# Danderson123/Amira

Measured on AMD Instinct MI355X. Metric: gene-mers/s to corrected GeneMerGraph, higher is better.
Workload: dtype int32; 1 GPU; synthetic 1M reads x 60 genes, k=5, 20k-gene vocab: build + error-correction sweep (build, filter(3,1), correct, build, clip(5), correct, build); reads_per_gpu=1000000, genes_per_read=60, k=5, vocab=20000, gene_mers_per_gpu=56000000, final_nodes=472478, final_edges=1054844, multi_gpu=n/a

## Files before the change

amira_amd/csrc/amg_scan.hip:

```cpp
#include "amg_rows.h"

#define SC_THREADS 512
#define SC_ROWS 16
#define SC_TILE (SC_THREADS * SC_ROWS)
#define SC_VAL_MASK ((1ull << 48) - 1ull)

__device__ __forceinline__ unsigned long long sc_word(unsigned int state, unsigned int epoch, unsigned long long v) {
  return ((unsigned long long)state << 62) | ((unsigned long long)(epoch & 0x3fffu) << 48) | (v & SC_VAL_MASK);
}

#define SC_NO_LIM 0x7fffffffffffffffll
template <class T>
struct LoadArr {
  const T* in;
  using Raw = T;
  __device__ __forceinline__ long long lim() const { return SC_NO_LIM; }
  __device__ __forceinline__ Raw raw(long long i) const { return in[i]; }
  __device__ __forceinline__ unsigned long long val(long long, Raw r) const { return (unsigned long long)r; }
};
template <class T>
struct LoadArrN {
  const T* in;
  long long n;
  using Raw = T;
  __device__ __forceinline__ long long lim() const { return n; }
  __device__ __forceinline__ Raw raw(long long i) const { return in[i]; }
  __device__ __forceinline__ unsigned long long val(long long, Raw r) const { return (unsigned long long)r; }
};
struct LoadNonzero {
  const unsigned int* in;
  long long n;
  using Raw = unsigned int;
  __device__ __forceinline__ long long lim() const { return n; }
  __device__ __forceinline__ Raw raw(long long i) const { return in[i]; }
  __device__ __forceinline__ unsigned long long val(long long, Raw r) const { return r != 0u ? 1ull : 0ull; }
};
struct LoadByteSet {
  const unsigned char* in;
  long long n;
  using Raw = unsigned char;
  __device__ __forceinline__ long long lim() const { return n; }
  __device__ __forceinline__ Raw raw(long long i) const { return in[i]; }
  __device__ __forceinline__ unsigned long long val(long long, Raw r) const { return r != 0 ? 1ull : 0ull; }
};
struct LoadApplyKill {
  unsigned char* kill;
  unsigned char* alive;
  long long n;
  struct Raw {
    unsigned int kill, alive;
  };
  __device__ __forceinline__ long long lim() const { return n; }
  __device__ __forceinline__ Raw raw(long long i) const { return Raw{kill[i], alive[i]}; }
  __device__ __forceinline__ unsigned long long val(long long i, Raw r) const {
    const bool f = r.kill != 0u && r.alive != 0u;
    if (f) alive[i] = 0;
    kill[i] = f ? 1 : 0;
    return f ? 1ull : 0ull;
  }
};
struct LoadFlagWords {
  const unsigned char* flags;
  unsigned int* bits;
  long long n_words;
  struct Raw {
    uint4 a, b;
  };
  __device__ __forceinline__ long long lim() const { return n_words; }
  __device__ __forceinline__ Raw raw(long long i) const {
    const uint4* p = reinterpret_cast<const uint4*>(flags + 32 * i);
    return Raw{p[0], p[1]};
  }
  __device__ __forceinline__ unsigned long long val(long long i, const Raw& r) const {
    auto nib = [](unsigned int x) { return (x & 1u) | ((x >> 7) & 2u) | ((x >> 14) & 4u) | ((x >> 21) & 8u); };
    const uint4 a = r.a, b = r.b;
    const unsigned int w = nib(a.x) | (nib(a.y) << 4) | (nib(a.z) << 8) | (nib(a.w) << 12) | (nib(b.x) << 16) |
                           (nib(b.y) << 20) | (nib(b.z) << 24) | (nib(b.w) << 28);
    bits[i] = w;
    return (unsigned long long)__popc(w);
  }
};
struct LoadBitsPopc {
  const unsigned int* bits;
  long long n_words;
  using Raw = unsigned int;
  __device__ __forceinline__ long long lim() const { return n_words; }
  __device__ __forceinline__ Raw raw(long long i) const { return bits[i]; }
  __device__ __forceinline__ unsigned long long val(long long, Raw r) const { return (unsigned long long)__popc(r); }
};
struct LoadPairWidth {
  const unsigned long long* pkey;
  long long n_pairs;
  using Raw = unsigned long long;
  __device__ __forceinline__ long long lim() const { return n_pairs; }
  __device__ __forceinline__ Raw raw(long long i) const { return pkey[i]; }
  __device__ __forceinline__ unsigned long long val(long long, Raw key) const {
    const unsigned int lo = (unsigned int)((key >> 32) & 0x7fffffffull);
    const unsigned int hi = (unsigned int)(key & 0xffffffffull) - 1u;
    return lo == hi ? 1ull : 2ull;
  }
};

struct LoadNone {
  using Raw = unsigned char;
  __device__ __forceinline__ long long lim() const { return 0; }
  __device__ __forceinline__ Raw raw(long long) const { return 0; }
  __device__ __forceinline__ unsigned long long val(long long, Raw) const { return 0ull; }
};

template <class L>
__device__ __forceinline__ void load_rows(const L& ld, long long w0, long long n, int lane, unsigned long long* x) {
  const long long lim = n < ld.lim() ? n : ld.lim();
  if (w0 >= lim) {
#pragma unroll
    for (int r = 0; r < SC_ROWS; ++r) x[r] = 0ull;
    return;
  }
  typename L::Raw raw[SC_ROWS];
#pragma unroll
  for (int r = 0; r < SC_ROWS; ++r) {
    const long long i = w0 + r * 64 + lane;
    raw[r] = ld.raw(i < lim ? i : lim - 1);
  }
  asm volatile("" ::: "memory");
#pragma unroll
  for (int r = 0; r < SC_ROWS; ++r) {
    const long long i = w0 + r * 64 + lane;
    x[r] = i < lim ? ld.val(i, raw[r]) : 0ull;
  }
}

struct EmitOut {
  long long* out;
  struct Pre {};
  __device__ __forceinline__ Pre pre(long long) const { return Pre{}; }
  __device__ __forceinline__ void operator()(long long i, unsigned long long excl, const Pre&, unsigned long long) const {
    out[i] = (long long)excl;
  }
};
struct EmitEdges {
  const unsigned long long* pkey;
  const unsigned int* pcnt;
  const unsigned long long* pfirst;
  long long n_pairs;
  long long* total;
  int* e_src;
  int* e_tgt;
  signed char* e_sdir;
  signed char* e_tdir;
  unsigned int* e_cov;
  unsigned char* e_alive;
  struct Pre {
    unsigned long long key, first;
    unsigned int cnt;
  };
  __device__ __forceinline__ Pre pre(long long i) const {
    const long long j = i < n_pairs ? i : 0;
    return Pre{pkey[j], pfirst[j], pcnt[j]};
  }
  __device__ __forceinline__ void operator()(long long i, unsigned long long excl, const Pre& p, unsigned long long) const {
    if (i >= n_pairs) {
      total[0] = (long long)excl;
      return;
    }
    const unsigned long long key = p.key, first = p.first;
    const int lo = (int)((key >> 32) & 0x7fffffffull);
    const int hi = (int)((key & 0xffffffffull) - 1ull);
    const int X = (first & 1ull) ? lo : hi, Y = (first & 1ull) ? hi : lo;
    const signed char dX = (first & 2ull) ? 1 : -1, dY = (first & 4ull) ? 1 : -1;
    const long long e = (long long)excl;
    const unsigned int cnt = p.cnt;
    e_src[e] = X; e_tgt[e] = Y; e_sdir[e] = dX; e_tdir[e] = dY; e_alive[e] = 1;
    if (lo == hi) {
      e_cov[e] = cnt * 2u;
    } else {
      e_cov[e] = cnt;
      e_src[e + 1] = Y; e_tgt[e + 1] = X; e_sdir[e + 1] = (signed char)-dY;
      e_tdir[e + 1] = (signed char)-dX; e_cov[e + 1] = cnt; e_alive[e + 1] = 1;
    }
  }
};
struct EmitLiveKeys {
  const int* e_src;
  const signed char* e_sdir;
  long long n_edges;
  long long* total;
  unsigned int* keys;
  unsigned int* edge_of;
  struct Pre {};
  __device__ __forceinline__ Pre pre(long long) const { return Pre{}; }
  __device__ __forceinline__ void operator()(long long i, unsigned long long excl, const Pre&, unsigned long long val) const {
    if (i >= n_edges) {
      total[0] = (long long)excl;
      return;
    }
    if (val == 0ull) return;
    keys[excl] = adj_row_of(e_src[i], e_sdir[i]);
    edge_of[excl] = (unsigned int)i;
  }
};
template <class Load, class LoadB, class Emit>
__global__ __launch_bounds__(SC_THREADS) void k_exscan(Load load, Emit emit_a, long long n_a, LoadB load_b,
                                                        long long* __restrict__ out_b, long long n_b, long long tiles_a,
                                                        unsigned long long* counter, unsigned long long ticket_base,
                                                        unsigned long long* status, unsigned int epoch, ClearArgs side) {
  __shared__ unsigned long long s_wave[SC_THREADS / 64];
  __shared__ unsigned long long s_excl;
  __shared__ unsigned int s_tile;
  const int lane = threadIdx.x & 63, wave = threadIdx.x >> 6;
  if (threadIdx.x == 0) s_tile = (unsigned int)(atomicAdd(counter, 1ull) - ticket_base);
  __syncthreads();
  const long long tile = s_tile;
  const bool second = tile >= tiles_a;
  const long long seg0 = second ? tiles_a : 0;
  const long long n = second ? n_b : n_a;
  const long long w0 = (tile - seg0) * SC_TILE + (long long)wave * (64 * SC_ROWS);
  unsigned long long x[SC_ROWS], inc[SC_ROWS];
  if (second)
    load_rows(load_b, w0, n, lane, x);
  else
    load_rows(load, w0, n, lane, x);
  unsigned long long row_off = 0;
#pragma unroll
  for (int r = 0; r < SC_ROWS; ++r) {
    unsigned long long v = x[r];
#pragma unroll
    for (int d = 1; d < 64; d <<= 1) {
      const unsigned long long o = __shfl_up(v, d, 64);
      if (lane >= d) v += o;
    }
    inc[r] = v + row_off;
    row_off += __shfl(v, 63, 64);
  }
  if (lane == 0) s_wave[wave] = row_off;
  __syncthreads();
  unsigned long long wave_excl = 0, tile_sum = 0;
#pragma unroll
  for (int w = 0; w < SC_THREADS / 64; ++w) {
    const unsigned long long s = s_wave[w];
    wave_excl += w < wave ? s : 0ull;
    tile_sum += s;
  }
  typename Emit::Pre pre[SC_ROWS];
  if (!second) {
#pragma unroll
    for (int r = 0; r < SC_ROWS; ++r) {
      const long long i = w0 + r * 64 + lane;
      pre[r] = emit_a.pre(i < n ? i : n - 1);
    }
  }
  if (wave == 0) {
    unsigned long long excl = 0;
    if (tile == seg0) {
      if (lane == 0)
        __hip_atomic_store(status + tile, sc_word(2u, epoch, tile_sum), __ATOMIC_RELAXED, __HIP_MEMORY_SCOPE_AGENT);
    } else {
      if (lane == 0)
        __hip_atomic_store(status + tile, sc_word(1u, epoch, tile_sum), __ATOMIC_RELAXED, __HIP_MEMORY_SCOPE_AGENT);
      for (long long look = tile - 1;; look -= 64) {
        const long long idx = look - lane;
        unsigned int state = 2u;
        unsigned long long val = 0;
        if (idx >= seg0) {
          unsigned long long w;
          do {
            w = __hip_atomic_load(status + idx, __ATOMIC_RELAXED, __HIP_MEMORY_SCOPE_AGENT);
          } while ((unsigned int)((w >> 48) & 0x3fffu) != (epoch & 0x3fffu) || (w >> 62) == 0ull);
          state = (unsigned int)(w >> 62);
          val = w & SC_VAL_MASK;
        }
        const unsigned long long full = __ballot(state == 2u);
        const int stop = full ? __ffsll((long long)full) - 1 : 63;
        unsigned long long part = lane <= stop ? val : 0ull;
#pragma unroll
        for (int d = 32; d > 0; d >>= 1) part += __shfl_xor(part, d, 64);
        excl += part;
        if (full) break;
      }
      if (lane == 0)
        __hip_atomic_store(status + tile, sc_word(2u, epoch, excl + tile_sum), __ATOMIC_RELAXED, __HIP_MEMORY_SCOPE_AGENT);
    }
    if (lane == 0) s_excl = excl;
  }
  __syncthreads();
  const unsigned long long base = s_excl + wave_excl;
#pragma unroll
  for (int r = 0; r < SC_ROWS; ++r) {
    const long long i = w0 + r * 64 + lane;
    if (i < n) {
      if (second)
        out_b[i] = (long long)(base + inc[r] - x[r]);
      else
        emit_a(i, base + inc[r] - x[r], pre[r], x[r]);
    }
  }
  if (side.n) clear_args_part(side, blockIdx.x, gridDim.x);
}

template <class Load, class Emit, class LoadB = LoadNone>
static int exscan_emit(amg_ctx* c, Load load, Emit emit, size_t n, LoadB load_b = LoadNone{}, long long* out_b = nullptr,
                       size_t n_b = 0, const ClearList* side = nullptr) {
  if (side && side->overflow) return amg_fail(AMG_E_ARG, "exscan: more than %d ranges in one list", CLEAR_MAX);
  if (n == 0 && n_b == 0) return side ? clear_many(c, *side) : AMG_OK;
  const unsigned long long tiles_a = (n + SC_TILE - 1) / SC_TILE;
  const unsigned long long tiles = tiles_a + (n_b + SC_TILE - 1) / SC_TILE;
  const size_t need = (size_t)(tiles + 8) * sizeof(unsigned long long);
  if (need > c->scan_state.cap || c->scan_epoch >= 0x3fffu) {
    if (need > c->scan_state.cap) {
      AMGCHK(c->scan_state.ensure(need * 2));
      c->scan_tickets = 0;
      HIPCHK(hipMemsetAsync(c->scan_state.p, 0, c->scan_state.cap, c->stream));
    } else {
      HIPCHK(hipMemsetAsync(c->scan_state.as<unsigned long long>() + 8, 0,
                            c->scan_state.cap - 8 * sizeof(unsigned long long), c->stream));
    }
    c->scan_epoch = 0;
  }
  const unsigned int epoch = ++c->scan_epoch;
  unsigned long long* st = c->scan_state.as<unsigned long long>();
  ClearArgs sa;
  sa.n = 0;
  if (side) sa = clear_args(*side);
  hipLaunchKernelGGL((k_exscan<Load, LoadB, Emit>), dim3((unsigned int)tiles), dim3(SC_THREADS), 0, c->stream, load, emit,
                     (long long)n, load_b, out_b, (long long)n_b, (long long)tiles_a, st, c->scan_tickets, st + 8, epoch, sa);
  c->scan_tickets += tiles;
  return AMG_OK;
}

template <class Load, class LoadB = LoadNone>
static int exscan(amg_ctx* c, Load load, long long* out, size_t n, LoadB load_b = LoadNone{}, long long* out_b = nullptr,
                  size_t n_b = 0) {
  return exscan_emit(c, load, EmitOut{out}, n, load_b, out_b, n_b);
}

int prim_exscan_u32_to_i64(amg_ctx* c, const unsigned int* in, long long* out, size_t n) {
  return exscan(c, LoadArr<unsigned int>{in}, out, n);
}

int prim_exscan_i64(amg_ctx* c, const long long* in, long long* out, size_t n) {
  return exscan(c, LoadArr<long long>{in}, out, n);
}

int prim_exscan_u32_pair(amg_ctx* c, const unsigned int* in_a, long long* out_a, const unsigned int* in_b, long long* out_b,
                         size_t n) {
  return exscan(c, LoadArrN<unsigned int>{in_a, (long long)n}, out_a, n + 1, LoadArrN<unsigned int>{in_b, (long long)n}, out_b,
                n + 1);
}

int prim_exscan_i64_pair(amg_ctx* c, const long long* in_a, long long* out_a, const long long* in_b, long long* out_b,
                         size_t n) {
  return exscan(c, LoadArrN<long long>{in_a, (long long)n}, out_a, n + 1, LoadArrN<long long>{in_b, (long long)n}, out_b,
                n + 1);
}

int prim_exscan_bytes_set(amg_ctx* c, const unsigned char* in, long long* out, size_t n, const ClearList* side) {
  return exscan_emit(c, LoadByteSet{in, (long long)n}, EmitOut{out}, n + 1, LoadNone{}, nullptr, 0, side);
}

int prim_exscan_apply_kill(amg_ctx* c, unsigned char* kill, unsigned char* alive, long long* out, size_t n) {
  return exscan(c, LoadApplyKill{kill, alive, (long long)n}, out, n + 1);
}

int prim_exscan_keep_and_len(amg_ctx* c, const unsigned int* len, long long* out_keep, long long* out_off, size_t n) {
  return exscan(c, LoadNonzero{len, (long long)n}, out_keep, n + 1, LoadArrN<unsigned int>{len, (long long)n}, out_off, n + 1);
}

int prim_exscan_flag_words(amg_ctx* c, const unsigned char* flags, unsigned int* bits, long long* out, size_t n_words) {
  return exscan(c, LoadFlagWords{flags, bits, (long long)n_words}, out, n_words + 1);
}

int prim_exscan_bits_popc(amg_ctx* c, const unsigned int* bits, long long* out, size_t n_words) {
  return exscan(c, LoadBitsPopc{bits, (long long)n_words}, out, n_words + 1);
}

int prim_exscan_pair_width(amg_ctx* c, const unsigned long long* pkey, long long* out, size_t n_pairs) {
  return exscan(c, LoadPairWidth{pkey, (long long)n_pairs}, out, n_pairs + 1);
}

int prim_exscan_emit_edges(amg_ctx* c, const unsigned long long* pkey, const unsigned int* pcnt,
                           const unsigned long long* pfirst, size_t n_pairs, long long* total, int* e_src, int* e_tgt,
                           signed char* e_sdir, signed char* e_tdir, unsigned int* e_cov, unsigned char* e_alive,
                           const ClearList* side) {
  return exscan_emit(c, LoadPairWidth{pkey, (long long)n_pairs},
                     EmitEdges{pkey, pcnt, pfirst, (long long)n_pairs, total, e_src, e_tgt, e_sdir, e_tdir, e_cov, e_alive},
                     n_pairs + 1, LoadNone{}, nullptr, 0, side);
}

int prim_exscan_live_edges(amg_ctx* c, const unsigned char* e_alive, const int* e_src, const signed char* e_sdir, size_t n_edges,
                           long long* total, unsigned int* keys, unsigned int* edge_of, const ClearList* side) {
  return exscan_emit(c, LoadByteSet{e_alive, (long long)n_edges},
                     EmitLiveKeys{e_src, e_sdir, (long long)n_edges, total, keys, edge_of}, n_edges + 1, LoadNone{}, nullptr, 0,
                     side);
}

extern "C" int amg_scan_probe(amg_ctx* c, int kind, const void* in, int64_t n, int64_t* out, void* aux) {
  if (!c || n < 0 || (n > 0 && !in) || !out) return amg_fail(AMG_E_ARG, "scan_probe: bad arguments");
  size_t in_bytes = 0, out_words = (size_t)n + 1, aux_bytes = 0;
  switch (kind) {
    case 0: in_bytes = (size_t)n; aux_bytes = (size_t)n; break;
    case 1: in_bytes = 8 * (size_t)n; break;
    case 2: in_bytes = 32 * (size_t)n; aux_bytes = 4 * (size_t)n; break;
    case 3: in_bytes = 2 * (size_t)n; aux_bytes = 2 * (size_t)n; break;
    case 4: in_bytes = 4 * (size_t)n; out_words = 2 * ((size_t)n + 1); break;
    case 5: in_bytes = 20 * (size_t)n; out_words = 1; aux_bytes = 30 * (size_t)n; break;
    case 6: in_bytes = 6 * (size_t)n; out_words = 1; aux_bytes = 8 * (size_t)n; break;
    default: return amg_fail(AMG_E_ARG, "scan_probe: unknown kind %d", kind);
  }
  char* d = nullptr;
  const size_t in_cap = (in_bytes + 255) & ~(size_t)255, out_cap = (out_words * 8 + 255) & ~(size_t)255;
  const size_t aux_cap = (aux_bytes + 256) & ~(size_t)255;
  HIPCHK(hipMalloc(reinterpret_cast<void**>(&d), in_cap + out_cap + aux_cap));
  char* din = d;
  long long* dout = reinterpret_cast<long long*>(d + in_cap);
  char* daux = d + in_cap + out_cap;
  int rc = AMG_OK;
  do {
    if (in_bytes && hipMemcpy(din, in, in_bytes, hipMemcpyHostToDevice) != hipSuccess) { rc = amg_fail(AMG_E_HIP, "h2d"); break; }
    if (hipMemset(daux, 0xff, aux_cap) != hipSuccess || hipDeviceSynchronize() != hipSuccess) {
      rc = amg_fail(AMG_E_HIP, "memset");
      break;
    }
    switch (kind) {
      case 0: {
        ClearList side;
        side.add(daux, (size_t)n);
        rc = prim_exscan_bytes_set(c, reinterpret_cast<unsigned char*>(din), dout, (size_t)n, &side);
        break;
      }
      case 1: rc = prim_exscan_pair_width(c, reinterpret_cast<unsigned long long*>(din), dout, (size_t)n); break;
      case 2:
        rc = prim_exscan_flag_words(c, reinterpret_cast<unsigned char*>(din), reinterpret_cast<unsigned int*>(daux), dout,
                                    (size_t)n);
        break;
      case 3:
        if (n && (hipMemcpy(daux, din, 2 * (size_t)n, hipMemcpyDeviceToDevice) != hipSuccess ||
                  hipDeviceSynchronize() != hipSuccess)) {
          rc = amg_fail(AMG_E_HIP, "d2d");
          break;
        }
        rc = prim_exscan_apply_kill(c, reinterpret_cast<unsigned char*>(daux), reinterpret_cast<unsigned char*>(daux) + n,
                                    dout, (size_t)n);
        break;
      case 4:
        rc = prim_exscan_keep_and_len(c, reinterpret_cast<unsigned int*>(din), dout, dout + n + 1, (size_t)n);
        break;
      case 5: {
        const size_t E = 2 * (size_t)n;
        int* src = reinterpret_cast<int*>(daux);
        int* tgt = src + E;
        unsigned int* cov = reinterpret_cast<unsigned int*>(tgt + E);
        signed char* sdir = reinterpret_cast<signed char*>(cov + E);
        signed char* tdir = sdir + E;
        unsigned char* alive = reinterpret_cast<unsigned char*>(tdir + E);
        rc = prim_exscan_emit_edges(c, reinterpret_cast<unsigned long long*>(din),
                                    reinterpret_cast<unsigned int*>(din + 16 * (size_t)n),
                                    reinterpret_cast<unsigned long long*>(din + 8 * (size_t)n), (size_t)n, dout, src, tgt,
                                    sdir, tdir, cov, alive, nullptr);
        break;
      }
      case 6: {
        unsigned int* keys = reinterpret_cast<unsigned int*>(daux);
        rc = prim_exscan_live_edges(c, reinterpret_cast<unsigned char*>(din + 4 * (size_t)n), reinterpret_cast<int*>(din),
                                    reinterpret_cast<signed char*>(din + 5 * (size_t)n), (size_t)n, dout, keys, keys + n,
                                    nullptr);
        break;
      }
    }
    if (rc != AMG_OK) break;
    if (hipStreamSynchronize(c->stream) != hipSuccess) { rc = amg_fail(AMG_E_HIP, "scan_probe: stream"); break; }
    if (hipMemcpy(out, dout, out_words * 8, hipMemcpyDeviceToHost) != hipSuccess) { rc = amg_fail(AMG_E_HIP, "d2h"); break; }
    if (aux && aux_bytes && hipMemcpy(aux, daux, aux_bytes, hipMemcpyDeviceToHost) != hipSuccess) { rc = amg_fail(AMG_E_HIP, "d2h"); break; }
  } while (false);
  (void)hipFree(d);
  return rc;
}
```

Measured before the change: 10.34 billion gene-mers/s.

## Vectorize decoupled-lookback scan loads with per-type packed elements and alignment-aware tiling

```diff
diff --git a/amira_amd/csrc/amg_scan.hip b/amira_amd/csrc/amg_scan.hip
--- a/amira_amd/csrc/amg_scan.hip
+++ b/amira_amd/csrc/amg_scan.hip
@@ -1,8 +1,8 @@
+#include <type_traits>
+
 #include "amg_rows.h"
 
 #define SC_THREADS 512
-#define SC_ROWS 16
-#define SC_TILE (SC_THREADS * SC_ROWS)
 #define SC_VAL_MASK ((1ull << 48) - 1ull)
 
 __device__ __forceinline__ unsigned long long sc_word(unsigned int state, unsigned int epoch, unsigned long long v) {
@@ -10,127 +10,329 @@
 }
 
 #define SC_NO_LIM 0x7fffffffffffffffll
+
+__device__ __forceinline__ bool sc_in(long long i, long long lim) { return (unsigned long long)i < (unsigned long long)lim; }
+__device__ __forceinline__ long long sc_clamp(long long i, long long lim) { return i < 0 ? 0 : (i < lim ? i : lim - 1); }
 template <class T>
-struct LoadArr {
+__host__ __device__ __forceinline__ int sc_mis(const T* p, int e) {
+  return (int)(((unsigned long long)reinterpret_cast<uintptr_t>(p) / sizeof(T)) % (unsigned int)e);
+}
+__device__ __forceinline__ unsigned int sc_nz_bytes(unsigned int w) {
+  return ((((w & 0x7f7f7f7fu) + 0x7f7f7f7fu) | w) & 0x80808080u) >> 7;
+}
+
+template <class T, int E_>
+struct alignas(sizeof(T) * E_) ScPack {
+  T v[E_];
+};
+template <class T, int E_>
+__device__ __forceinline__ ScPack<T, E_> sc_pack_vec(const T* in, long long i0) {
+  return *reinterpret_cast<const ScPack<T, E_>*>(in + i0);
+}
+template <class T, int E_>
+__device__ __forceinline__ ScPack<T, E_> sc_pack_elems(const T* in, long long i0, long long lim) {
+  ScPack<T, E_> p;
+#pragma unroll
+  for (int j = 0; j < E_; ++j) p.v[j] = in[sc_clamp(i0 + j, lim)];
+  return p;
+}
+template <bool FULL, class T, int E_>
+__device__ __forceinline__ ScPack<T, E_> sc_pack_mask(const ScPack<T, E_>& r, long long i0, long long lim) {
+  ScPack<T, E_> k;
+#pragma unroll
+  for (int j = 0; j < E_; ++j) k.v[j] = (FULL || sc_in(i0 + j, lim)) ? r.v[j] : (T)0;
+  return k;
+}
+
+template <class L>
+__device__ __forceinline__ typename L::Sum sc_sum_at(const typename L::Keep& k) {
+  typename L::Sum s = 0;
+#pragma unroll
+  for (int j = 0; j < L::E; ++j) s += (typename L::Sum)L::at(k, j);
+  return s;
+}
+
+template <class T>
+struct ScArr {
+  static constexpr int E = 16 / (int)sizeof(T), ROWS = 16 / E, BATCH = ROWS;
+  using Raw = ScPack<T, E>;
+  using Keep = Raw;
   const T* in;
-  using Raw = T;
+  __host__ __device__ __forceinline__ int mis() const { return sc_mis(in, E); }
+  __device__ __forceinline__ bool vec() const { return true; }
+  __device__ __forceinline__ Raw raw_vec(long long i0) const { return sc_pack_vec<T, E>(in, i0); }
+  __device__ __forceinline__ Raw raw_elems(long long i0, long long lim) const { return sc_pack_elems<T, E>(in, i0, lim); }
+  template <bool FULL>
+  __device__ __forceinline__ Keep keep(long long i0, long long lim, const Raw& r) const {
+    return sc_pack_mask<FULL>(r, i0, lim);
+  }
+};
+template <class T>
+struct LoadArr : ScArr<T> {
+  using Sum = unsigned long long;
+  using Keep = typename ScArr<T>::Keep;
+  __host__ __device__ LoadArr(const T* p) : ScArr<T>{p} {}
   __device__ __forceinline__ long long lim() const { return SC_NO_LIM; }
-  __device__ __forceinline__ Raw raw(long long i) const { return in[i]; }
-  __device__ __forceinline__ unsigned long long val(long long, Raw r) const { return (unsigned long long)r; }
+  static __device__ __forceinline__ unsigned long long at(const Keep& k, int j) { return (unsigned long long)k.v[j]; }
+  static __device__ __forceinline__ Sum sum(const Keep& k) { return sc_sum_at<LoadArr<T>>(k); }
 };
 template <class T>
-struct LoadArrN {
-  const T* in;
+struct LoadArrN : ScArr<T> {
+  using Sum = unsigned long long;
+  using Keep = typename ScArr<T>::Keep;
   long long n;
-  using Raw = T;
+  __host__ __device__ LoadArrN(const T* p, long long n_) : ScArr<T>{p}, n(n_) {}
   __device__ __forceinline__ long long lim() const { return n; }
-  __device__ __forceinline__ Raw raw(long long i) const { return in[i]; }
-  __device__ __forceinline__ unsigned long long val(long long, Raw r) const { return (unsigned long long)r; }
-};
-struct LoadNonzero {
-  const unsigned int* in;
+  static __device__ __forceinline__ unsigned long long at(const Keep& k, int j) { return (unsigned long long)k.v[j]; }
+  static __device__ __forceinline__ Sum sum(const Keep& k) { return sc_sum_at<LoadArrN<T>>(k); }
+};
+struct LoadNonzero : ScArr<unsigned int> {
+  using Sum = unsigned int;
   long long n;
-  using Raw = unsigned int;
+  __host__ __device__ LoadNonzero(const unsigned int* p, long long n_) : ScArr<unsigned int>{p}, n(n_) {}
   __device__ __forceinline__ long long lim() const { return n; }
-  __device__ __forceinline__ Raw raw(long long i) const { return in[i]; }
-  __device__ __forceinline__ unsigned long long val(long long, Raw r) const { return r != 0u ? 1ull : 0ull; }
+  static __device__ __forceinline__ unsigned long long at(const Keep& k, int j) { return k.v[j] != 0u ? 1ull : 0ull; }
+  static __device__ __forceinline__ Sum sum(const Keep& k) { return sc_sum_at<LoadNonzero>(k); }
+};
+struct LoadBitsPopc : ScArr<unsigned int> {
+  using Sum = unsigned int;
+  long long n_words;
+  __host__ __device__ LoadBitsPopc(const unsigned int* p, long long n_) : ScArr<unsigned int>{p}, n_words(n_) {}
+  __device__ __forceinline__ long long lim() const { return n_words; }
+  static __device__ __forceinline__ unsigned long long at(const Keep& k, int j) { return (unsigned long long)__popc(k.v[j]); }
+  static __device__ __forceinline__ Sum sum(const Keep& k) { return sc_sum_at<LoadBitsPopc>(k); }
+};
+template <int E_>
+struct LoadPairWidth {
+  static constexpr int E = E_, ROWS = 16 / E_, BATCH = ROWS;
+  using Sum = unsigned int;
+  using Raw = ScPack<unsigned long long, E_>;
+  struct Keep {
+    unsigned int v[E_];
+  };
+  const unsigned long long* pkey;
+  long long n_pairs;
+  __device__ __forceinline__ long long lim() const { return n_pairs; }
+  __host__ __device__ __forceinline__ int mis() const { return sc_mis(pkey, E); }
+  __device__ __forceinline__ bool vec() const { return true; }
+  __device__ __forceinline__ Raw raw_vec(long long i0) const { return sc_pack_vec<unsigned long long, E_>(pkey, i0); }
+  __device__ __forceinline__ Raw raw_elems(long long i0, long long lim) const {
+    return sc_pack_elems<unsigned long long, E_>(pkey, i0, lim);
+  }
+  template <bool FULL>
+  __device__ __forceinline__ Keep keep(long long i0, long long lim, const Raw& r) const {
+    Keep k;
+#pragma unroll
+    for (int j = 0; j < E_; ++j) {
+      const unsigned long long key = r.v[j];
+      const unsigned int lo = (unsigned int)((key >> 32) & 0x7fffffffull);
+      const unsigned int hi = (unsigned int)(key & 0xffffffffull) - 1u;
+      k.v[j] = (FULL || sc_in(i0 + j, lim)) ? (lo == hi ? 1u : 2u) : 0u;
+    }
+    return k;
+  }
+  static __device__ __forceinline__ unsigned long long at(const Keep& k, int j) { return (unsigned long long)k.v[j]; }
+  static __device__ __forceinline__ Sum sum(const Keep& k) { return sc_sum_at<LoadPairWidth<E_>>(k); }
 };
 struct LoadByteSet {
+  static constexpr int E = 16, ROWS = 2, BATCH = ROWS;
+  using Sum = unsigned int;
+  struct Raw {
+    unsigned int w[4];
+  };
+  using Keep = Raw;
   const unsigned char* in;
   long long n;
-  using Raw = unsigned char;
   __device__ __forceinline__ long long lim() const { return n; }
-  __device__ __forceinline__ Raw raw(long long i) const { return in[i]; }
-  __device__ __forceinline__ unsigned long long val(long long, Raw r) const { return r != 0 ? 1ull : 0ull; }
+  __host__ __device__ __forceinline__ int mis() const { return sc_mis(in, E); }
+  __device__ __forceinline__ bool vec() const { return true; }
+  __device__ __forceinline__ Raw raw_vec(long long i0) const {
+    const uint4 q = *reinterpret_cast<const uint4*>(in + i0);
+    return Raw{{q.x, q.y, q.z, q.w}};
+  }
+  __device__ __forceinline__ Raw raw_elems(long long i0, long long lim) const {
+    unsigned int b[16];
+#pragma unroll
+    for (int j = 0; j < 16; ++j) b[j] = in[sc_clamp(i0 + j, lim)];
+    Raw r;
+#pragma unroll
+    for (int q = 0; q < 4; ++q) r.w[q] = b[4 * q] | (b[4 * q + 1] << 8) | (b[4 * q + 2] << 16) | (b[4 * q + 3] << 24);
+    return r;
+  }
+  template <bool FULL>
+  __device__ __forceinline__ Keep keep(long long i0, long long lim, const Raw& r) const {
+    Keep k;
+#pragma unroll
+    for (int q = 0; q < 4; ++q) {
+      unsigned int m = 0xffffffffu;
+      if (!FULL) {
+        m = 0u;
+#pragma unroll
+        for (int j = 0; j < 4; ++j) m |= sc_in(i0 + 4 * q + j, lim) ? 0xffu << (8 * j) : 0u;
+      }
+      k.w[q] = sc_nz_bytes(r.w[q] & m);
+    }
+    return k;
+  }
+  static __device__ __forceinline__ unsigned long long at(const Keep& k, int j) {
+    return (unsigned long long)((k.w[j >> 2] >> (8 * (j & 3))) & 1u);
+  }
+  static __device__ __forceinline__ Sum sum(const Keep& k) { return (Sum)(__popc(k.w[0]) + __popc(k.w[1]) + __popc(k.w[2]) + __popc(k.w[3])); }
 };
 struct LoadApplyKill {
+  static constexpr int E = 8, ROWS = 2, BATCH = ROWS;
+  using Sum = unsigned int;
+  struct Raw {
+    unsigned int kill[2], alive[2];
+  };
+  struct Keep {
+    unsigned int w[2];
+  };
   unsigned char* kill;
   unsigned char* alive;
   long long n;
-  struct Raw {
-    unsigned int kill, alive;
-  };
   __device__ __forceinline__ long long lim() const { return n; }
-  __device__ __forceinline__ Raw raw(long long i) const { return Raw{kill[i], alive[i]}; }
-  __device__ __forceinline__ unsigned long long val(long long i, Raw r) const {
-    const bool f = r.kill != 0u && r.alive != 0u;
-    if (f) alive[i] = 0;
-    kill[i] = f ? 1 : 0;
-    return f ? 1ull : 0ull;
-  }
+  __host__ __device__ __forceinline__ int mis() const { return sc_mis(kill, E); }
+  __device__ __forceinline__ bool vec() const {
+    return ((reinterpret_cast<uintptr_t>(kill) ^ reinterpret_cast<uintptr_t>(alive)) & 7u) == 0u;
+  }
+  __device__ __forceinline__ Raw raw_vec(long long i0) const {
+    const uint2 k = *reinterpret_cast<const uint2*>(kill + i0), a = *reinterpret_cast<const uint2*>(alive + i0);
+    return Raw{{k.x, k.y}, {a.x, a.y}};
+  }
+  __device__ __forceinline__ Raw raw_elems(long long i0, long long lim) const {
+    unsigned int k[8], a[8];
+#pragma unroll
+    for (int j = 0; j < 8; ++j) {
+      const long long i = sc_clamp(i0 + j, lim);
+      k[j] = kill[i];
+      a[j] = alive[i];
+    }
+    Raw r;
+#pragma unroll
+    for (int q = 0; q < 2; ++q) {
+      r.kill[q] = k[4 * q] | (k[4 * q + 1] << 8) | (k[4 * q + 2] << 16) | (k[4 * q + 3] << 24);
+      r.alive[q] = a[4 * q] | (a[4 * q + 1] << 8) | (a[4 * q + 2] << 16) | (a[4 * q + 3] << 24);
+    }
+    return r;
+  }
+  template <bool FULL>
+  __device__ __forceinline__ Keep keep(long long i0, long long lim, const Raw& r) const {
+    Keep f;
+#pragma unroll
+    for (int q = 0; q < 2; ++q) f.w[q] = sc_nz_bytes(r.kill[q]) & sc_nz_bytes(r.alive[q]);
+    if (FULL) {
+      *reinterpret_cast<uint2*>(kill + i0) = uint2{f.w[0], f.w[1]};
+      if (f.w[0] | f.w[1])
+        *reinterpret_cast<uint2*>(alive + i0) = uint2{r.alive[0] & ~(f.w[0] * 0xffu), r.alive[1] & ~(f.w[1] * 0xffu)};
+    } else {
+#pragma unroll
+      for (int j = 0; j < 8; ++j) {
+        const unsigned int sh = 8u * (unsigned int)(j & 3);
+        if (sc_in(i0 + j, lim)) {
+          const bool d = ((f.w[j >> 2] >> sh) & 1u) != 0u;
+          if (d) alive[i0 + j] = 0;
+          kill[i0 + j] = d ? 1 : 0;
+        } else {
+          f.w[j >> 2] &= ~(0xffu << sh);
+        }
+      }
+    }
+    return f;
+  }
+  static __device__ __forceinline__ unsigned long long at(const Keep& k, int j) {
+    return (unsigned long long)((k.w[j >> 2] >> (8 * (j & 3))) & 1u);
+  }
+  static __device__ __forceinline__ Sum sum(const Keep& k) { return (Sum)(__popc(k.w[0]) + __popc(k.w[1])); }
 };
 struct LoadFlagWords {
+  static constexpr int E = 2, ROWS = 8, BATCH = 8;
+  using Sum = unsigned int;
   const unsigned char* flags;
   unsigned int* bits;
   long long n_words;
   struct Raw {
-    uint4 a, b;
+    uint4 q[4];
+  };
+  struct Keep {
+    unsigned int w[2];
   };
   __device__ __forceinline__ long long lim() const { return n_words; }
-  __device__ __forceinline__ Raw raw(long long i) const {
-    const uint4* p = reinterpret_cast<const uint4*>(flags + 32 * i);
-    return Raw{p[0], p[1]};
-  }
-  __device__ __forceinline__ unsigned long long val(long long i, const Raw& r) const {
+  __host__ __device__ __forceinline__ int mis() const { return 0; }
+  __device__ __forceinline__ bool vec() const { return true; }
+  __device__ __forceinline__ Raw raw_vec(long long i0) const {
+    const uint4* p = reinterpret_cast<const uint4*>(flags + 32 * i0);
+    return Raw{{p[0], p[1], p[2], p[3]}};
+  }
+  __device__ __forceinline__ Raw raw_elems(long long i0, long long lim) const {
+    const uint4* p0 = reinterpret_cast<const uint4*>(flags + 32 * sc_clamp(i0, lim));
+    const uint4* p1 = reinterpret_cast<const uint4*>(flags + 32 * sc_clamp(i0 + 1, lim));
+    return Raw{{p0[0], p0[1], p1[0], p1[1]}};
+  }
+  template <bool FULL>
+  __device__ __forceinline__ Keep keep(long long i0, long long lim, const Raw& r) const {
     auto nib = [](unsigned int x) { return (x & 1u) | ((x >> 7) & 2u) | ((x >> 14) & 4u) | ((x >> 21) & 8u); };
-    const uint4 a = r.a, b = r.b;
-    const unsigned int w = nib(a.x) | (nib(a.y) << 4) | (nib(a.z) << 8) | (nib(a.w) << 12) | (nib(b.x) << 16) |
-                           (nib(b.y) << 20) | (nib(b.z) << 24) | (nib(b.w) << 28);
-    bits[i] = w;
-    return (unsigned long long)__popc(w);
-  }
-};
-struct LoadBitsPopc {
-  const unsigned int* bits;
-  long long n_words;
-  using Raw = unsigned int;
-  __device__ __forceinline__ long long lim() const { return n_words; }
-  __device__ __forceinline__ Raw raw(long long i) const { return bits[i]; }
-  __device__ __forceinline__ unsigned long long val(long long, Raw r) const { return (unsigned long long)__popc(r); }
-};
-struct LoadPairWidth {
-  const unsigned long long* pkey;
-  long long n_pairs;
-  using Raw = unsigned long long;
-  __device__ __forceinline__ long long lim() const { return n_pairs; }
-  __device__ __forceinline__ Raw raw(long long i) const { return pkey[i]; }
-  __device__ __forceinline__ unsigned long long val(long long, Raw key) const {
-    const unsigned int lo = (unsigned int)((key >> 32) & 0x7fffffffull);
-    const unsigned int hi = (unsigned int)(key & 0xffffffffull) - 1u;
-    return lo == hi ? 1ull : 2ull;
-  }
+    Keep k;
+#pragma unroll
+    for (int j = 0; j < 2; ++j) {
+      const uint4 a = r.q[2 * j], b = r.q[2 * j + 1];
+      const unsigned int w = nib(a.x) | (nib(a.y) << 4) | (nib(a.z) << 8) | (nib(a.w) << 12) | (nib(b.x) << 16) |
+                             (nib(b.y) << 20) | (nib(b.z) << 24) | (nib(b.w) << 28);
+      k.w[j] = (FULL || sc_in(i0 + j, lim)) ? w : 0u;
+      if (FULL || sc_in(i0 + j, lim)) bits[i0 + j] = w;
+    }
+    return k;
+  }
+  static __device__ __forceinline__ unsigned long long at(const Keep& k, int j) { return (unsigned long long)__popc(k.w[j]); }
+  static __device__ __forceinline__ Sum sum(const Keep& k) { return (Sum)(__popc(k.w[0]) + __popc(k.w[1])); }
 };
 
 struct LoadNone {
-  using Raw = unsigned char;
-  __device__ __forceinline__ long long lim() const { return 0; }
-  __device__ __forceinline__ Raw raw(long long) const { return 0; }
-  __device__ __forceinline__ unsigned long long val(long long, Raw) const { return 0ull; }
+  static constexpr int E = 1, ROWS = 1, BATCH = 1;
+  __host__ __device__ __forceinline__ int mis() const { return 0; }
 };
 
 template <class L>
-__device__ __forceinline__ void load_rows(const L& ld, long long w0, long long n, int lane, unsigned long long* x) {
+struct ScTile {
+  static constexpr long long N = (long long)SC_THREADS * L::ROWS * L::E;
+};
+
+template <class L>
+__device__ __forceinline__ void load_rows(const L& ld, long long wi0, long long n, int lane, typename L::Keep* keep) {
+  constexpr int E = L::E, ROWS = L::ROWS, BATCH = L::BATCH;
   const long long lim = n < ld.lim() ? n : ld.lim();
-  if (w0 >= lim) {
-#pragma unroll
-    for (int r = 0; r < SC_ROWS; ++r) x[r] = 0ull;
+  if (lim <= 0 || wi0 >= lim) {
+#pragma unroll
+    for (int r = 0; r < ROWS; ++r) keep[r] = typename L::Keep{};
     return;
   }
-  typename L::Raw raw[SC_ROWS];
-#pragma unroll
-  for (int r = 0; r < SC_ROWS; ++r) {
-    const long long i = w0 + r * 64 + lane;
-    raw[r] = ld.raw(i < lim ? i : lim - 1);
-  }
-  asm volatile("" ::: "memory");
-#pragma unroll
-  for (int r = 0; r < SC_ROWS; ++r) {
-    const long long i = w0 + r * 64 + lane;
-    x[r] = i < lim ? ld.val(i, raw[r]) : 0ull;
+  const bool full = ld.vec() && wi0 >= 0 && wi0 + 64ll * E * ROWS <= lim;
+  if (full) {
+#pragma unroll
+    for (int b = 0; b < ROWS; b += BATCH) {
+      typename L::Raw raw[BATCH];
+#pragma unroll
+      for (int r = 0; r < BATCH; ++r) raw[r] = ld.raw_vec(wi0 + (long long)((b + r) * 64 + lane) * E);
+      asm volatile("" ::: "memory");
+#pragma unroll
+      for (int r = 0; r < BATCH; ++r)
+        keep[b + r] = ld.template keep<true>(wi0 + (long long)((b + r) * 64 + lane) * E, lim, raw[r]);
+      asm volatile("" ::: "memory");
+    }
+  } else {
+#pragma unroll
+    for (int r = 0; r < ROWS; ++r) {
+      const long long i0 = wi0 + (long long)(r * 64 + lane) * E;
+      const typename L::Raw raw = ld.raw_elems(i0, lim);
+      asm volatile("" ::: "memory");
+      keep[r] = ld.template keep<false>(i0, lim, raw);
+      asm volatile("" ::: "memory");
+    }
   }
 }
 
 struct EmitOut {
+  static constexpr bool OUT = true, WAVE = false;
   long long* out;
   struct Pre {};
   __device__ __forceinline__ Pre pre(long long) const { return Pre{}; }
@@ -139,6 +341,7 @@
   }
 };
 struct EmitEdges {
+  static constexpr bool OUT = false, WAVE = false;
   const unsigned long long* pkey;
   const unsigned int* pcnt;
   const unsigned long long* pfirst;
@@ -180,7 +383,9 @@
     }
   }
 };
+#define SC_LIVE_DENSE 64
 struct EmitLiveKeys {
+  static constexpr bool OUT = false, WAVE = true;
   const int* e_src;
   const signed char* e_sdir;
   long long n_edges;
@@ -189,50 +394,115 @@
   unsigned int* edge_of;
   struct Pre {};
   __device__ __forceinline__ Pre pre(long long) const { return Pre{}; }
-  __device__ __forceinline__ void operator()(long long i, unsigned long long excl, const Pre&, unsigned long long val) const {
-    if (i >= n_edges) {
-      total[0] = (long long)excl;
-      return;
-    }
-    if (val == 0ull) return;
-    keys[excl] = adj_row_of(e_src[i], e_sdir[i]);
-    edge_of[excl] = (unsigned int)i;
-  }
-};
-template <class Load, class LoadB, class Emit>
-__global__ __launch_bounds__(SC_THREADS) void k_exscan(Load load, Emit emit_a, long long n_a, LoadB load_b,
-                                                        long long* __restrict__ out_b, long long n_b, long long tiles_a,
-                                                        unsigned long long* counter, unsigned long long ticket_base,
-                                                        unsigned long long* status, unsigned int epoch, ClearArgs side) {
-  __shared__ unsigned long long s_wave[SC_THREADS / 64];
-  __shared__ unsigned long long s_excl;
-  __shared__ unsigned int s_tile;
-  const int lane = threadIdx.x & 63, wave = threadIdx.x >> 6;
-  if (threadIdx.x == 0) s_tile = (unsigned int)(atomicAdd(counter, 1ull) - ticket_base);
-  __syncthreads();
-  const long long tile = s_tile;
-  const bool second = tile >= tiles_a;
-  const long long seg0 = second ? tiles_a : 0;
-  const long long n = second ? n_b : n_a;
-  const long long w0 = (tile - seg0) * SC_TILE + (long long)wave * (64 * SC_ROWS);
-  unsigned long long x[SC_ROWS], inc[SC_ROWS];
-  if (second)
-    load_rows(load_b, w0, n, lane, x);
-  else
-    load_rows(load, w0, n, lane, x);
-  unsigned long long row_off = 0;
-#pragma unroll
-  for (int r = 0; r < SC_ROWS; ++r) {
-    unsigned long long v = x[r];
+  template <int ROWS>
+  static __device__ __forceinline__ unsigned int pick(const unsigned int* a, int r) {
+    unsigned int x = a[0];
+#pragma unroll
+    for (int k = 1; k < ROWS; ++k) x = r == k ? a[k] : x;
+    return x;
+  }
+  template <int ROWS>
+  __device__ __forceinline__ void wave(long long wi0, int lane, unsigned long long base, const unsigned int* lane_excl,
+                                       const LoadByteSet::Keep* keep) const {
+    static_assert(ROWS <= 8, "the lane's elements are kept as two 64-bit masks");
+    auto nib = [](unsigned int w) { return ((w * 0x01020408u) >> 24) & 0xfu; };
+    unsigned int m[ROWS];
+#pragma unroll
+    for (int r = 0; r < ROWS; ++r)
+      m[r] = nib(keep[r].w[0]) | (nib(keep[r].w[1]) << 4) | (nib(keep[r].w[2]) << 8) | (nib(keep[r].w[3]) << 12);
+    const long long t = n_edges - wi0;
+    if (t >= 0 && t < 1024ll * ROWS) {
+      const int tr = (int)(t >> 10), tj = (int)t & 15;
+      if (lane == ((int)(t >> 4) & 63))
+        total[0] = (long long)(base + pick<ROWS>(lane_excl, tr) + __popc(pick<ROWS>(m, tr) & ((1u << tj) - 1u)));
+    }
+    unsigned long long q[2] = {0ull, 0ull};
+#pragma unroll
+    for (int r = 0; r < ROWS; ++r) {
+      const unsigned int live = __builtin_amdgcn_readlane(lane_excl[r] + __popc(m[r]), 63) -
+                                __builtin_amdgcn_readlane(lane_excl[r], 0);
+      if (live < SC_LIVE_DENSE) {
+        q[r >> 2] |= (unsigned long long)m[r] << (16 * (r & 3));
+        continue;
+      }
+      const long long i0 = wi0 + (long long)(r * 64 + lane) * 16;
+      int s[16];
+      signed char d[16];
+#pragma unroll
+      for (int j = 0; j < 16; ++j) {
+        const long long i = sc_clamp(i0 + j, n_edges);
+        s[j] = e_src[i];
+        d[j] = e_sdir[i];
+      }
+      unsigned long long at = base + lane_excl[r];
+#pragma unroll
+      for (int j = 0; j < 16; ++j) {
+        if ((m[r] >> j) & 1u) {
+          keys[at] = adj_row_of(s[j], d[j]);
+          edge_of[at] = (unsigned int)(i0 + j);
+          ++at;
+        }
+      }
+    }
+    while (__ballot((q[0] | q[1]) != 0ull)) {
+      long long idx[2];
+      unsigned long long at[2];
+      bool ok[2];
+#pragma unroll
+      for (int u = 0; u < 2; ++u) {
+        const bool lo = q[0] != 0ull;
+        const unsigned long long w = lo ? q[0] : q[1];
+        ok[u] = w != 0ull;
+        const int pos = ok[u] ? __ffsll((long long)w) - 1 + (lo ? 0 : 64) : 0;
+        if (lo) q[0] &= q[0] - 1ull; else q[1] &= q[1] - 1ull;
+        const int r = pos >> 4, j = pos & 15;
+        idx[u] = wi0 + (long long)(r * 64 + lane) * 16 + j;
+        at[u] = base + pick<ROWS>(lane_excl, r) + __popc(pick<ROWS>(m, r) & ((1u << j) - 1u));
+      }
+      int s[2];
+      signed char d[2];
+#pragma unroll
+      for (int u = 0; u < 2; ++u) {
+        const long long i = ok[u] ? idx[u] : 0;
+        s[u] = e_src[i];
+        d[u] = e_sdir[i];
+      }
+#pragma unroll
+      for (int u = 0; u < 2; ++u) {
+        if (ok[u]) {
+          keys[at[u]] = adj_row_of(s[u], d[u]);
+          edge_of[at[u]] = (unsigned int)idx[u];
+        }
+      }
+    }
+  }
+};
+
+template <class L, class Emit>
+__device__ __forceinline__ void scan_tile(const L& ld, const Emit& emit, long long n, long long tile, long long seg0,
+                                          unsigned long long* status, unsigned int epoch, unsigned long long* s_wave,
+                                          unsigned long long* s_excl) {
+  constexpr int E = L::E, ROWS = L::ROWS;
+  using Sum = typename L::Sum;
+  const int lane = threadIdx.x & 63, wave = __builtin_amdgcn_readfirstlane(threadIdx.x >> 6);
+  const long long wi0 = (tile - seg0) * ScTile<L>::N + (long long)wave * (64 * E * ROWS) - ld.mis();
+  typename L::Keep keep[ROWS];
+  load_rows(ld, wi0, n, lane, keep);
+  Sum lane_excl[ROWS];
+  Sum row_off = 0;
+#pragma unroll
+  for (int r = 0; r < ROWS; ++r) {
+    const Sum s = L::sum(keep[r]);
+    Sum v = s;
 #pragma unroll
     for (int d = 1; d < 64; d <<= 1) {
-      const unsigned long long o = __shfl_up(v, d, 64);
+      const Sum o = __shfl_up(v, d, 64);
       if (lane >= d) v += o;
     }
-    inc[r] = v + row_off;
+    lane_excl[r] = v - s + row_off;
     row_off += __shfl(v, 63, 64);
   }
-  if (lane == 0) s_wave[wave] = row_off;
+  if (lane == 0) s_wave[wave] = (unsigned long long)row_off;
   __syncthreads();
   unsigned long long wave_excl = 0, tile_sum = 0;
 #pragma unroll
@@ -241,13 +511,12 @@
     wave_excl += w < wave ? s : 0ull;
     tile_sum += s;
   }
-  typename Emit::Pre pre[SC_ROWS];
-  if (!second) {
-#pragma unroll
-    for (int r = 0; r < SC_ROWS; ++r) {
-      const long long i = w0 + r * 64 + lane;
-      pre[r] = emit_a.pre(i < n ? i : n - 1);
-    }
+  typename Emit::Pre pre[ROWS][E];
+#pragma unroll
+  for (int r = 0; r < ROWS; ++r) {
+#pragma unroll
+    for (int j = 0; j < E; ++j)
+      pre[r][j] = emit.pre(sc_clamp(wi0 + (long long)(r * 64 + lane) * E + j, n));
   }
   if (wave == 0) {
     unsigned long long excl = 0;
@@ -280,21 +549,69 @@
       if (lane == 0)
         __hip_atomic_store(status + tile, sc_word(2u, epoch, excl + tile_sum), __ATOMIC_RELAXED, __HIP_MEMORY_SCOPE_AGENT);
     }
-    if (lane == 0) s_excl = excl;
+    if (lane == 0) *s_excl = excl;
   }
   __syncthreads();
-  const unsigned long long base = s_excl + wave_excl;
-#pragma unroll
-  for (int r = 0; r < SC_ROWS; ++r) {
-    const long long i = w0 + r * 64 + lane;
-    if (i < n) {
-      if (second)
-        out_b[i] = (long long)(base + inc[r] - x[r]);
-      else
-        emit_a(i, base + inc[r] - x[r], pre[r], x[r]);
-    }
+  const unsigned long long base = *s_excl + wave_excl;
+  if constexpr (Emit::WAVE) {
+    emit.template wave<ROWS>(wi0, lane, base, lane_excl, keep);
+  } else {
+    bool pairs = false;
+    if constexpr (Emit::OUT) pairs = (reinterpret_cast<uintptr_t>(emit.out + wi0) & 15u) == 0u;
+#pragma unroll
+    for (int r = 0; r < ROWS; ++r) {
+      const long long i0 = wi0 + (long long)(r * 64 + lane) * E;
+      unsigned long long p[E];
+      unsigned long long run = base + (unsigned long long)lane_excl[r];
+#pragma unroll
+      for (int j = 0; j < E; ++j) {
+        p[j] = run;
+        run += L::at(keep[r], j);
+      }
+      bool done = false;
+      if constexpr (Emit::OUT && E % 2 == 0) {
+        if (pairs && i0 >= 0 && i0 + E <= n) {
+#pragma unroll
+          for (int j = 0; j < E; j += 2)
+            *reinterpret_cast<ulonglong2*>(emit.out + i0 + j) = ulonglong2{p[j], p[j + 1]};
+          done = true;
+        }
+      }
+      if (!done) {
+#pragma unroll
+        for (int j = 0; j < E; ++j)
+          if (sc_in(i0 + j, n)) emit(i0 + j, p[j], pre[r][j], L::at(keep[r], j));
+      }
+      __builtin_amdgcn_sched_barrier(0);
+    }
+  }
+}
+
+template <class Load, class LoadB, class Emit>
+__global__ __launch_bounds__(SC_THREADS) void k_exscan(Load load, Emit emit_a, long long n_a, LoadB load_b,
+                                                        long long* __restrict__ out_b, long long n_b, long long tiles_a,
+                                                        unsigned long long* counter, unsigned long long ticket_base,
+                                                        unsigned long long* status, unsigned int epoch, ClearArgs side) {
+  __shared__ unsigned long long s_wave[SC_THREADS / 64];
+  __shared__ unsigned long long s_excl;
+  __shared__ unsigned int s_tile;
+  if (threadIdx.x == 0) s_tile = (unsigned int)(atomicAdd(counter, 1ull) - ticket_base);
+  __syncthreads();
+  const long long tile = s_tile;
+  if constexpr (!std::is_same<LoadB, LoadNone>::value) {
+    if (tile >= tiles_a)
+      scan_tile(load_b, EmitOut{out_b}, n_b, tile, tiles_a, status, epoch, s_wave, &s_excl);
+    else
+      scan_tile(load, emit_a, n_a, tile, 0, status, epoch, s_wave, &s_excl);
+  } else {
+    scan_tile(load, emit_a, n_a, tile, 0, status, epoch, s_wave, &s_excl);
   }
   if (side.n) clear_args_part(side, blockIdx.x, gridDim.x);
+}
+
+template <class L>
+static unsigned long long scan_tiles(const L& ld, size_t n) {
+  return n ? ((unsigned long long)n + (unsigned long long)ld.mis() + ScTile<L>::N - 1) / ScTile<L>::N : 0ull;
 }
 
 template <class Load, class Emit, class LoadB = LoadNone>
@@ -302,8 +619,8 @@
                        size_t n_b = 0, const ClearList* side = nullptr) {
   if (side && side->overflow) return amg_fail(AMG_E_ARG, "exscan: more than %d ranges in one list", CLEAR_MAX);
   if (n == 0 && n_b == 0) return side ? clear_many(c, *side) : AMG_OK;
-  const unsigned long long tiles_a = (n + SC_TILE - 1) / SC_TILE;
-  const unsigned long long tiles = tiles_a + (n_b + SC_TILE - 1) / SC_TILE;
+  const unsigned long long tiles_a = scan_tiles(load, n);
+  const unsigned long long tiles = tiles_a + scan_tiles(load_b, n_b);
   const size_t need = (size_t)(tiles + 8) * sizeof(unsigned long long);
   if (need > c->scan_state.cap || c->scan_epoch >= 0x3fffu) {
     if (need > c->scan_state.cap) {
@@ -374,14 +691,14 @@
 }
 
 int prim_exscan_pair_width(amg_ctx* c, const unsigned long long* pkey, long long* out, size_t n_pairs) {
-  return exscan(c, LoadPairWidth{pkey, (long long)n_pairs}, out, n_pairs + 1);
+  return exscan(c, LoadPairWidth<2>{pkey, (long long)n_pairs}, out, n_pairs + 1);
 }
 
 int prim_exscan_emit_edges(amg_ctx* c, const unsigned long long* pkey, const unsigned int* pcnt,
                            const unsigned long long* pfirst, size_t n_pairs, long long* total, int* e_src, int* e_tgt,
                            signed char* e_sdir, signed char* e_tdir, unsigned int* e_cov, unsigned char* e_alive,
                            const ClearList* side) {
-  return exscan_emit(c, LoadPairWidth{pkey, (long long)n_pairs},
+  return exscan_emit(c, LoadPairWidth<1>{pkey, (long long)n_pairs},
                      EmitEdges{pkey, pcnt, pfirst, (long long)n_pairs, total, e_src, e_tgt, e_sdir, e_tdir, e_cov, e_alive},
                      n_pairs + 1, LoadNone{}, nullptr, 0, side);
 }
@@ -394,29 +711,54 @@
 }
 
 extern "C" int amg_scan_probe(amg_ctx* c, int kind, const void* in, int64_t n, int64_t* out, void* aux) {
-  if (!c || n < 0 || (n > 0 && !in) || !out) return amg_fail(AMG_E_ARG, "scan_probe: bad arguments");
-  size_t in_bytes = 0, out_words = (size_t)n + 1, aux_bytes = 0;
+  if (!c || kind < 0 || n < 0 || (n > 0 && !in) || !out) return amg_fail(AMG_E_ARG, "scan_probe: bad arguments");
+  const size_t mis = (size_t)((kind >> 8) & 0xff), mis_b = (size_t)((kind >> 16) & 0xff);
+  if ((kind >> 24) || (mis_b && (kind & 0xff) != 7)) return amg_fail(AMG_E_ARG, "scan_probe: bad misalignment bits");
+  kind &= 0xff;
+  size_t in_bytes = 0, out_words = (size_t)n + 1, aux_bytes = 0, elem = 1;
   switch (kind) {
     case 0: in_bytes = (size_t)n; aux_bytes = (size_t)n; break;
-    case 1: in_bytes = 8 * (size_t)n; break;
-    case 2: in_bytes = 32 * (size_t)n; aux_bytes = 4 * (size_t)n; break;
+    case 1: in_bytes = 8 * (size_t)n; elem = 8; break;
+    case 2: in_bytes = 32 * (size_t)n; aux_bytes = 4 * (size_t)n; elem = 32; break;
     case 3: in_bytes = 2 * (size_t)n; aux_bytes = 2 * (size_t)n; break;
-    case 4: in_bytes = 4 * (size_t)n; out_words = 2 * ((size_t)n + 1); break;
-    case 5: in_bytes = 20 * (size_t)n; out_words = 1; aux_bytes = 30 * (size_t)n; break;
+    case 4: in_bytes = 4 * (size_t)n; out_words = 2 * ((size_t)n + 1); elem = 4; break;
+    case 5: in_bytes = 20 * (size_t)n; out_words = 1; aux_bytes = 30 * (size_t)n; elem = 8; break;
     case 6: in_bytes = 6 * (size_t)n; out_words = 1; aux_bytes = 8 * (size_t)n; break;
+    case 7: in_bytes = 8 * (size_t)n; out_words = 2 * ((size_t)n + 1); elem = 4; break;
     default: return amg_fail(AMG_E_ARG, "scan_probe: unknown kind %d", kind);
   }
+  const size_t shift = mis * elem;
+  if (shift > 256 || mis_b * elem > 256) return amg_fail(AMG_E_ARG, "scan_probe: misalignment of %zu bytes (256 at most)", shift);
   char* d = nullptr;
-  const size_t in_cap = (in_bytes + 255) & ~(size_t)255, out_cap = (out_words * 8 + 255) & ~(size_t)255;
-  const size_t aux_cap = (aux_bytes + 256) & ~(size_t)255;
+  const size_t in_cap = ((in_bytes + 255) & ~(size_t)255) + 768, out_cap = (out_words * 8 + 255) & ~(size_t)255;
+  const size_t aux_cap = ((aux_bytes + 256) & ~(size_t)255) + 256;
   HIPCHK(hipMalloc(reinterpret_cast<void**>(&d), in_cap + out_cap + aux_cap));
-  char* din = d;
+  char* din = d + (kind == 3 || kind == 6 ? 0 : shift);
   long long* dout = reinterpret_cast<long long*>(d + in_cap);
-  char* daux = d + in_cap + out_cap;
+  char* daux = d + in_cap + out_cap + (kind == 3 ? shift : 0);
+  char* dalive = d + ((4 * (size_t)n + 255) & ~(size_t)255) + shift;
+  char* dsecond = d + ((shift + 4 * (size_t)n + 255) & ~(size_t)255) + mis_b * elem;
   int rc = AMG_OK;
   do {
-    if (in_bytes && hipMemcpy(din, in, in_bytes, hipMemcpyHostToDevice) != hipSuccess) { rc = amg_fail(AMG_E_HIP, "h2d"); break; }
-    if (hipMemset(daux, 0xff, aux_cap) != hipSuccess || hipDeviceSynchronize() != hipSuccess) {
+    if (kind == 6 && n) {
+      const char* h = static_cast<const char*>(in);
+      if (hipMemcpy(din, h, 4 * (size_t)n, hipMemcpyHostToDevice) != hipSuccess ||
+          hipMemcpy(dalive, h + 4 * (size_t)n, 2 * (size_t)n, hipMemcpyHostToDevice) != hipSuccess) {
+        rc = amg_fail(AMG_E_HIP, "h2d");
+        break;
+      }
+    } else if (kind == 7 && n) {
+      const char* h = static_cast<const char*>(in);
+      if (hipMemcpy(din, h, 4 * (size_t)n, hipMemcpyHostToDevice) != hipSuccess ||
+          hipMemcpy(dsecond, h + 4 * (size_t)n, 4 * (size_t)n, hipMemcpyHostToDevice) != hipSuccess) {
+        rc = amg_fail(AMG_E_HIP, "h2d");
+        break;
+      }
+    } else if (in_bytes && hipMemcpy(din, in, in_bytes, hipMemcpyHostToDevice) != hipSuccess) {
+      rc = amg_fail(AMG_E_HIP, "h2d");
+      break;
+    }
+    if (hipMemset(d + in_cap + out_cap, 0xff, aux_cap) != hipSuccess || hipDeviceSynchronize() != hipSuccess) {
       rc = amg_fail(AMG_E_HIP, "memset");
       break;
     }
@@ -460,11 +802,15 @@
       }
       case 6: {
         unsigned int* keys = reinterpret_cast<unsigned int*>(daux);
-        rc = prim_exscan_live_edges(c, reinterpret_cast<unsigned char*>(din + 4 * (size_t)n), reinterpret_cast<int*>(din),
-                                    reinterpret_cast<signed char*>(din + 5 * (size_t)n), (size_t)n, dout, keys, keys + n,
+        rc = prim_exscan_live_edges(c, reinterpret_cast<unsigned char*>(dalive), reinterpret_cast<int*>(din),
+                                    reinterpret_cast<signed char*>(dalive + (size_t)n), (size_t)n, dout, keys, keys + n,
                                     nullptr);
         break;
       }
+      case 7:
+        rc = prim_exscan_u32_pair(c, reinterpret_cast<unsigned int*>(din), dout, reinterpret_cast<unsigned int*>(dsecond),
+                                  dout + n + 1, (size_t)n);
+        break;
     }
     if (rc != AMG_OK) break;
     if (hipStreamSynchronize(c->stream) != hipSuccess) { rc = amg_fail(AMG_E_HIP, "scan_probe: stream"); break; }
```

New measurement: 10.47 billion gene-mers/s (median of 6 runs). 1.01x the previous value.
